# dfdazac/mpqe

Hardware: AMD Instinct MI355X
Metric: query-graphs/sec (encoder fwd+bwd) (higher is better)
Workload: dtype f32; 1 GPU; AIFB-shaped full query mix: 11 batches x B=512 per step (1/2/3-chain, 2x each of 2-inter, 3-inter, 3-inter_chain, 3-chain_inter), embed_dim=128, readout=mp, adaptive=True, num_layers=3 unshared, KG aifb (2601 entities, 89 typed relations); parallelism=single GPU

## Files before the change

### mpqe_amd/csrc/step.hip

```cpp
#include <stdio.h>
#include <stdlib.h>
#include <string.h>

#include <algorithm>
#include <memory>
#include <mutex>
#include <unordered_map>
#include <vector>

#include "grad_w_dma.h"
#include "rgcn_template_body.h"

#define STEP_MAX_LEVELS MPQE_STEP_MAX_LAYERS
#define CHAIN_MAX_GRAPHS (1 << 20)
#define UPLOAD_BYTES 2048

struct BatchDev {
    TmplArgs tp;
    int A, V, L, B;
    long long var_id[3];
    int anchor_tab[3];
    int target_tab;
    long long row_off, g_off, anchor_off;
    float weight;
// ... 956 lines not shown
__global__ __launch_bounds__(256) void adam_rows_kernel(const TouchHeader *__restrict__ th, const tkey_t *__restrict__ keys,
                                                        int D, RowAdamPtrs rp, float omb1, float omb2, float eps,
                                                        float neg_step_size, const int32_t *__restrict__ guard,
                                                        long long *__restrict__ applied) {
    if (guard && *guard != 0) return;
    if (applied && blockIdx.x == 0 && threadIdx.x == 0) *applied += 1;
    const int lpr = D / 4, per = 256 / lpr;
    const long long k = (long long)blockIdx.x * per + threadIdx.x / lpr;
    const int c = (threadIdx.x % lpr) * 4;
    if (k >= th->M) return;
    const tkey_t key = keys[k];
    if (key == TOUCH_INVALID || (k > 0 && keys[k - 1] == key)) return;
    const int tab = (int)(key >> th->row_bits);
    const long long off = (long long)(key & ((1ull << th->row_bits) - 1ull)) * D + c;
    float *p = rp.p[0], *m = rp.m[0], *v = rp.v[0];
    const float *g = rp.g[0];
#pragma unroll
    for (int t = 1; t < MPQE_STEP_MAX_MODES; ++t)
        if (t == tab) {
            p = rp.p[t];
            m = rp.m[t];
            v = rp.v[t];
            g = rp.g[t];
        }
    if (!p || !g || !m || !v) return;
    const f32x4 gg = gload4(g + off);
    f32x4 pp = *reinterpret_cast<f32x4 *>(p + off), mm = *reinterpret_cast<f32x4 *>(m + off);
    f32x4 vv = *reinterpret_cast<f32x4 *>(v + off);
#pragma unroll
    for (int e = 0; e < 4; ++e) {
        const float m_upd = __fmul_rn(__fsub_rn(gg[e], mm[e]), omb1);
        const float v_upd = __fmul_rn(__fsub_rn(__fmul_rn(gg[e], gg[e]), vv[e]), omb2);
        const float numer = __fadd_rn(m_upd, mm[e]);
        const float v_new = __fadd_rn(v_upd, vv[e]);
        const float denom = __fadd_rn(sqrtf(v_new), eps);
        mm[e] = __fadd_rn(mm[e], m_upd);
        vv[e] = v_new;
        pp[e] = __fadd_rn(pp[e], __fmul_rn(neg_step_size, __fdiv_rn(numer, denom)));
    }
    *reinterpret_cast<f32x4 *>(p + off) = pp;
    *reinterpret_cast<f32x4 *>(m + off) = mm;
    *reinterpret_cast<f32x4 *>(v + off) = vv;
}

extern "C" int64_t mpqe_step_touch_entries(const mpqe_step_batch_t *B, int nb) {
    if (!B || nb < 1 || nb > MPQE_STEP_MAX_BATCHES) return -1;
    return touch_entries(B, nb);
}

extern "C" size_t mpqe_rows_plan_bytes(int64_t n) { return n > 0 ? touch_layout(n, 0).total : 0; }
extern "C" size_t mpqe_rows_plan_workspace_bytes(int64_t n, int key_bits) {
    return n > 0 && key_bits > 0 && key_bits <= 64 ? touch_layout(n, key_bits).w_total : 0;
}
__global__ __launch_bounds__(256) void iota_kernel(int *__restrict__ v, long long n) {
    const long long i = (long long)blockIdx.x * 256 + threadIdx.x;
    if (i < n) v[i] = (int)i;
}
extern "C" int mpqe_rows_plan_build(const uint64_t *keys, int64_t n, int row_bits, int key_bits, void *plan,
                                    size_t plan_bytes, void *workspace, size_t workspace_bytes, void *stream) {
    if (!keys || !plan || !workspace || n <= 0 || n >= (1ll << 31) || row_bits <= 0 || key_bits <= row_bits || key_bits > 64)
        return MPQE_ERR_INVALID_ARG;
    const TouchLayout L = touch_layout(n, key_bits);
    if (plan_bytes < L.total || workspace_bytes < L.w_total) return MPQE_ERR_WORKSPACE;
    if ((uintptr_t)plan % 256 != 0 || (uintptr_t)workspace % 256 != 0) return MPQE_ERR_INVALID_ARG;
    hipStream_t s = as_stream(stream);
    char *tb = reinterpret_cast<char *>(plan), *wb = reinterpret_cast<char *>(workspace);
    TouchHeader th;
    memset(&th, 0, sizeof(th));
    th.M = n;
    th.row_bits = row_bits;
    th.key_bits = key_bits;
    upload(s, tb, &th, sizeof(th));
    int *vals = reinterpret_cast<int *>(wb + L.w_vals);
    hipLaunchKernelGGL(iota_kernel, dim3((unsigned)((n + 255) / 256)), dim3(256), 0, s, vals, (long long)n);
    if (radix_sort_pairs_own<tkey_t>(wb + L.w_tmp, reinterpret_cast<const tkey_t *>(keys), reinterpret_cast<tkey_t *>(tb + L.keys),
                                     (const int *)vals, reinterpret_cast<int *>(tb + L.perm), (long long)n, key_bits, s))
        return MPQE_ERR_LAUNCH;
    return mpqe_launch_status();
}
__global__ __launch_bounds__(256) void rows_sum_kernel(const char *__restrict__ plan, size_t o_keys, size_t o_perm,
                                                       const float *__restrict__ rows, int D, TablePtrs tabs, int store) {
    const TouchHeader *th = reinterpret_cast<const TouchHeader *>(plan);
    table_sum_block(th->M, th->row_bits, reinterpret_cast<const tkey_t *>(plan + o_keys),
                    reinterpret_cast<const int *>(plan + o_perm), rows, D, tabs, store, (long long)blockIdx.x);
}
extern "C" int mpqe_table_rows_sum(const void *plan, int64_t n, const float *rows, int64_t dim, float *const *table_grads,
                                   int num_modes, int store, void *stream) {
    if (!plan || !rows || !table_grads || n <= 0 || num_modes <= 0 || num_modes > MPQE_STEP_MAX_MODES)
        return MPQE_ERR_INVALID_ARG;
    if (dim <= 0 || dim % 4 != 0 || dim > 1024 || 256 % (dim / 4) != 0 || (uintptr_t)rows % 16 != 0) return MPQE_ERR_UNSUPPORTED;
    TablePtrs tabs;
    memset(&tabs, 0, sizeof(tabs));
    for (int m = 0; m < num_modes; ++m) {
        tabs.grad[m] = table_grads[m];
        if ((uintptr_t)table_grads[m] % 16 != 0) return MPQE_ERR_INVALID_ARG;
    }
    const TouchLayout L = touch_layout(n, 0);
    const long long per = 256 / (dim / 4);
    hipLaunchKernelGGL(rows_sum_kernel, dim3((unsigned)((n + per - 1) / per)), dim3(256), 0, as_stream(stream),
                       reinterpret_cast<const char *>(plan), L.keys, L.perm, rows, (int)dim, tabs, store);
    return mpqe_launch_status();
}

__global__ __launch_bounds__(256) void step_table_rows_kernel(const char *__restrict__ touch, size_t o_keys, size_t o_perm,
                                                              long long M, int row_bits, const float *__restrict__ DG, int D,
                                                              TablePtrs tabs, int store) {
    table_sum_block(M, row_bits, reinterpret_cast<const tkey_t *>(touch + o_keys), reinterpret_cast<const int *>(touch + o_perm),
                    DG, D, tabs, store, (long long)blockIdx.x, &reinterpret_cast<const TouchHeader *>(touch)->pad[0]);
}
extern "C" int mpqe_step_table_rows(const mpqe_step_params_t *P, const mpqe_step_batch_t *B, int nb, const mpqe_step_grads_t *G,
                                    const void *desc, void *workspace, size_t workspace_bytes, const void *touch, void *stream) {
    if (!P || !B || !G || !desc || !workspace || !touch || nb < 1 || nb > MPQE_STEP_MAX_BATCHES) return MPQE_ERR_INVALID_ARG;
    if ((uintptr_t)touch % 256 != 0 || (uintptr_t)workspace % 256 != 0) return MPQE_ERR_INVALID_ARG;
    std::shared_ptr<const CachedPlan> cached;
    if (plan_lookup(P, B, nb, nullptr, const_cast<void *>(desc), nullptr, &cached)) return MPQE_ERR_INVALID_ARG;
    const HostPlan &hp = cached->hp;
    if (!hp.chain || hp.touch_M <= 0) return MPQE_ERR_UNSUPPORTED;
    if (workspace_bytes < hp.total) return MPQE_ERR_WORKSPACE;
    const int D = P->dim;
    if (D % 4 != 0 || 256 % (D / 4) != 0) return MPQE_ERR_UNSUPPORTED;
    long long trows = 1;
    TablePtrs tabs;
    memset(&tabs, 0, sizeof(tabs));
    for (int m = 0; m < P->num_modes; ++m) {
        trows = std::max(trows, (long long)P->table_rows[m]);
        tabs.grad[m] = G->tables[m];
        tabs.rows[m] = P->table_rows[m];
        if (G->tables[m] && (uintptr_t)G->tables[m] % 16 != 0) return MPQE_ERR_INVALID_ARG;
    }
    const TouchLayout TL = touch_layout(hp.touch_M, 0);
    const long long per = 256 / (D / 4);
    const int store = ((P->flags & MPQE_STEP_SPARSE_TABLES) || (P->flags & MPQE_STEP_ZERO_GRADS)) ? 1 : 0;
    hipLaunchKernelGGL(step_table_rows_kernel, dim3((unsigned)((hp.touch_M + per - 1) / per)), dim3(256), 0, as_stream(stream),
                       reinterpret_cast<const char *>(touch), TL.keys, TL.perm, (long long)hp.touch_M, touch_bits(trows),
                       reinterpret_cast<const float *>(reinterpret_cast<const char *>(workspace) + hp.o_DG), D, tabs, store);
    return mpqe_launch_status();
}

static int adam_rows_launch(const void *touch, int64_t num_entries, float *const *params, const float *const *grads,
                            float *const *exp_avg, float *const *exp_avg_sq, int num_modes, int64_t dim, double lr,
                            double beta1, double beta2, double eps, int64_t step, const int32_t *guard, int64_t *applied,
                            void *stream) {
    if (!touch || num_entries <= 0 || !params || !grads || !exp_avg || !exp_avg_sq || step < 1) return MPQE_ERR_INVALID_ARG;
    if (num_modes <= 0 || num_modes > MPQE_STEP_MAX_MODES || dim <= 0 || dim % 4 != 0 || dim > 1024 || 256 % (dim / 4) != 0)
        return MPQE_ERR_UNSUPPORTED;
    if (!(beta1 >= 0. && beta1 < 1. && beta2 >= 0. && beta2 < 1.)) return MPQE_ERR_INVALID_ARG;
    const long long M = num_entries;
    RowAdamPtrs rp;
    memset(&rp, 0, sizeof(rp));
    for (int m = 0; m < num_modes; ++m) {
        rp.p[m] = params[m];
        rp.g[m] = grads[m];
        rp.m[m] = exp_avg[m];
        rp.v[m] = exp_avg_sq[m];
        if (((uintptr_t)rp.p[m] | (uintptr_t)rp.g[m] | (uintptr_t)rp.m[m] | (uintptr_t)rp.v[m]) % 16 != 0)
            return MPQE_ERR_INVALID_ARG;
    }
    const double bc1 = 1.0 - pow(beta1, (double)step), bc2 = 1.0 - pow(beta2, (double)step);
    const float neg_step = (float)(-(lr * sqrt(bc2) / bc1));
    const TouchLayout L = touch_layout(M, 0);
    const char *tb = reinterpret_cast<const char *>(touch);
    const long long per = 256 / (dim / 4);
    hipLaunchKernelGGL(adam_rows_kernel, dim3((unsigned)((M + per - 1) / per)), dim3(256), 0, as_stream(stream),
                       reinterpret_cast<const TouchHeader *>(tb), reinterpret_cast<const tkey_t *>(tb + L.keys), (int)dim, rp,
                       (float)(1.0 - beta1), (float)(1.0 - beta2), (float)eps, neg_step, guard,
                       reinterpret_cast<long long *>(applied));
    return mpqe_launch_status();
}

extern "C" int mpqe_adam_rows_step(const void *touch, int64_t num_entries, float *const *params,
                                   const float *const *grads, float *const *exp_avg, float *const *exp_avg_sq,
                                   int num_modes, int64_t dim, double lr, double beta1, double beta2, double eps,
                                   int64_t step, void *stream) {
    return adam_rows_launch(touch, num_entries, params, grads, exp_avg, exp_avg_sq, num_modes, dim, lr, beta1, beta2, eps,
                            step, nullptr, nullptr, stream);
}

extern "C" int mpqe_adam_rows_step_guarded(const void *touch, int64_t num_entries, float *const *params,
                                           const float *const *grads, float *const *exp_avg, float *const *exp_avg_sq,
                                           int num_modes, int64_t dim, double lr, double beta1, double beta2, double eps,
                                           int64_t step, const int32_t *guard, int64_t *applied, void *stream) {
    if (!guard) return MPQE_ERR_INVALID_ARG;
    return adam_rows_launch(touch, num_entries, params, grads, exp_avg, exp_avg_sq, num_modes, dim, lr, beta1, beta2, eps,
                            step, guard, applied, stream);
}

extern "C" int mpqe_l2_norms(const float *const *params, const int64_t *sizes, int count, const float *grad_out, float *out,
                             float *const *grads, void *stream) {
    if (!params || !sizes || count < 1 || count > 4 || (!out && !grads)) return MPQE_ERR_INVALID_ARG;
    RoRegArgs rr;
    memset(&rr, 0, sizeof(rr));
    for (int i = 0; i < count; ++i) {
        if (!params[i] || sizes[i] <= 0) return MPQE_ERR_INVALID_ARG;
        rr.p[i] = params[i];
        rr.n[i] = sizes[i];
        rr.g[i] = grads ? grads[i] : nullptr;
    }
    rr.coef = 1.f;
    rr.loss = out;
    rr.gscale = grad_out;
    hipLaunchKernelGGL(step_ro_reg_kernel, dim3(1), dim3(1024), 0, as_stream(stream), rr);
    return mpqe_launch_status();
}

static int D_ok_for_readout(int D) { return D % 4 == 0; }
static int readout_kin(const mpqe_step_params_t *P) {
    return P->readout == MPQE_READOUT_TARGETMLP ? 2 * P->dim : (P->readout == MPQE_READOUT_CONCAT ? P->num_layers * P->dim : P->dim);
}
// ... 42 lines not shown
```

### mpqe_amd/csrc/step_chain.h

```cpp
#pragma once
#include <type_traits>
#include "gemm_core.h"

#define CH_GB 16
#define CH_FIRST 1
#define CH_LAST 2
#define CH_LEVEL_END 4
#define CH_RELU 8
#define CH_MASK 16
#define CH_NOSTORE 32
#define CH_ADDG 64
#define CH_NOBIAS 128
#define CH_TSLOT_ON (1 << 20)
#define CH_MASK_LEVELS 4
#define CH_MAX_OPS 80
#define CH_MAX_CV 12

typedef float f32x2 __attribute__((ext_vector_type(2)));
typedef const f32x2 __attribute__((address_space(1))) * gvec2_ptr;
__device__ __forceinline__ f32x2 gload2(const float *p) { return *(gvec2_ptr)(p); }

struct ChainOp {
    unsigned char src, node, layer, level;
    int mat, flags;
// ... 964 lines not shown
#pragma unroll
            for (int cc = 0; cc < CC; ++cc) {
                q[cc] = h[A * CH_GB * LDX + sl + 16 * cc];
                arg[cc] = 0;
            }
        } else
#pragma unroll
        for (int cc = 0; cc < CC; ++cc) {
            const int col = sl + 16 * cc;
            float hn[4];
#pragma unroll
            for (int n = 0; n < 4; ++n) hn[n] = h[(n < N ? n : 0) * CH_GB * LDX + col];
            float sum = hn[0], best = hn[0];
            int am = 0;
#pragma unroll
            for (int n = 1; n < 4; ++n) {
                sum += n < N ? hn[n] : 0.f;
                const bool gt = n < N && hn[n] > best;
                best = gt ? hn[n] : best;
                am = gt ? n : am;
            }
            float tm = hn[0];
#pragma unroll
            for (int n = 1; n < 4; ++n) tm = n == A ? hn[n] : tm;
            q[cc] = readout == MPQE_READOUT_TM ? tm : (readout == MPQE_READOUT_SUM ? sum : best);
            arg[cc] = am;
        }
        if (ca.q_out && on) {
            float *qo = ca.q_out + (gi0 + i) * D;
#pragma unroll
            for (int cc = 0; cc < CC; ++cc) qo[sl + 16 * cc] = q[cc];
        }
        float ssp = 0.f, ssn = 0.f;
#pragma unroll
        for (int cc = 0; cc < CC; ++cc) {
            ssp += tp[cc] * tp[cc];
            ssn += tn[cc] * tn[cc];
        }
        ssp = gsum(ssp);
        ssn = gsum(ssn);
        const float ip0 = chain_rsq(ssp), in0 = chain_rsq(ssn);
        float dp = 0.f, dn = 0.f, qq = 0.f, pp = 0.f, nn = 0.f;
#pragma unroll
        for (int cc = 0; cc < CC; ++cc) {
            tp[cc] = pp_ ? tp[cc] * ip0 : 0.f;
            tn[cc] = pn_ ? tn[cc] * in0 : 0.f;
            dp += q[cc] * tp[cc];
            dn += q[cc] * tn[cc];
            qq += q[cc] * q[cc];
            pp += tp[cc] * tp[cc];
            nn += tn[cc] * tn[cc];
        }
        dp = gsum(dp);
        dn = gsum(dn);
        qq = gsum(qq);
        pp = gsum(pp);
        nn = gsum(nn);
        const float eps = ca.eps;
        const float rq = sqrtf(qq), rp = sqrtf(pp), rn = sqrtf(nn);
        const float nq = fmaxf(rq, eps), np_ = fmaxf(rp, eps), nn_ = fmaxf(rn, eps);
        const float sp = dp / (nq * np_), sn = dn / (nq * nn_);
        const float hv = ca.margin - (sp - sn);
        const long long gi = gi0 + i;
        const float term = on && hv > 0.f ? hv : 0.f;
        if (on && sl == 0) {
            ca.s_pos[gi] = sp;
            ca.s_neg[gi] = sn;
            ca.terms[gi] = term;
        }
        {
            float t4 = term + __shfl_xor(term, 16, 64);
            t4 += __shfl_xor(t4, 32, 64);
            if (lane == 0) S.red()[wave] = t4;
        }
        if (ca.backward) {
            const float act = hv >= 0.f ? b.weight / (float)b.B : 0.f;
            const float gsp = -act, gsn = act;
            const float inv_p = chain_rcp(nq * np_), inv_n = chain_rcp(nq * nn_);
            const float kq_ = rq > eps ? (gsp * sp + gsn * sn) * chain_rcp(nq * nq) : 0.f;
            const float ktp = rp > eps ? sp * chain_rcp(np_ * np_) : 0.f;
            const float ktn = rn > eps ? sn * chain_rcp(nn_ * nn_) : 0.f;
            const unsigned tmask = readout == MPQE_READOUT_SUM ? 0xFu : 1u << A;
            const unsigned liveL = b.live[RO ? L + 2 : L];
            float yg_p = 0.f, yg_n = 0.f;
#pragma unroll
            for (int cc = 0; cc < CC; ++cc) {
                const int col = sl + 16 * cc;
                const float gyp = gsp * (q[cc] * inv_p - ktp * tp[cc]);
                const float gyn = gsn * (q[cc] * inv_n - ktn * tn[cc]);
                yg_p += tp[cc] * gyp;
                yg_n += tn[cc] * gyn;
                float gq = gsp * tp[cc] * inv_p + gsn * tn[cc] * inv_n - kq_ * q[cc];
                if (RO) gq *= rscale;
                const unsigned takes = readout == MPQE_READOUT_MAX ? 1u << arg[cc] : tmask;
#pragma unroll
                for (int n = 0; n < 4; ++n) {
                    const float gv = (takes >> n) & 1u ? gq : 0.f;
                    if (n < N && ((liveL >> n) & 1u)) {
                        Xc[(n * CH_GB + i) * LDX + col] = gv;
                        if (on) GL[((long long)i * N + n) * D + col] = gv;
                    }
                }
            }
            yg_p = gsum(yg_p);
            yg_n = gsum(yg_n);
            float *gt = tabs.grad[b.target_tab];
            if (ca.DG && on) {
                float *dp_ = ca.DG + (ca.Manchor + ref.gi0 + i) * D, *dn_ = dp_ + ca.Gtot * D;
#pragma unroll
                for (int cc = 0; cc < CC; ++cc) {
                    const int col = sl + 16 * cc;
                    const float gyp = gsp * (q[cc] * inv_p - ktp * tp[cc]);
                    const float gyn = gsn * (q[cc] * inv_n - ktn * tn[cc]);
                    dp_[col] = pp_ ? (gyp - tp[cc] * yg_p) * ip0 : 0.f;
                    dn_[col] = pn_ ? (gyn - tn[cc] * yg_n) * in0 : 0.f;
                }
            } else if (gt && on) {
                const float *tb = tabs.table[b.target_tab];
#pragma unroll
                for (int cc = 0; cc < CC; ++cc) {
                    const int col = sl + 16 * cc;
                    const float gyp = gsp * (q[cc] * inv_p - ktp * tp[cc]);
                    const float gyn = gsn * (q[cc] * inv_n - ktn * tn[cc]);
                    if (CHAIN_DBG == 8) continue;
                    if (pp_) atomicAdd(gt + (pp_ - tb) + col, (gyp - tp[cc] * yg_p) * ip0);
                    if (pn_) atomicAdd(gt + (pn_ - tb) + col, (gyn - tn[cc] * yg_n) * in0);
                }
            }
        }
    }
    __syncthreads();
    if (tid == 0) {
        const float term = (S.red()[0] + S.red()[1]) + (S.red()[2] + S.red()[3]);
        if (ca.backward) ca.block_terms[ref.tb] = term;
        else agent_store(ca.block_terms + ref.tb, term);
    }
    if (!ca.backward) {
        chain_stamp(ca, 6);
        return;
    }
    chain_stamp(ca, 4);
    const int blk = g0 / CH_GB;
    for (int n = 0; n < N; ++n) {
        const int pr = b.lpart[n];
        if (pr < 0) continue;
        chain_colsum<NCB, KS, NW>(S, S.xs + cur * BUF, 1u << n, ng, ca.parts + (long long)(pr + blk) * D);
    }

    chain_run<NCB, KS, true, NW, RO>(S, nfwd, ref.bwd_count * IPO, N, ng, ca.GH + row0 * D, ca.level_stride, cur,
                                     ca.parts, blk);

    chain_stamp(ca, 5);
    if (ca.done) {
#ifndef MPQE_EMU
        asm volatile("s_waitcnt vmcnt(0)" ::: "memory");
#endif
        __syncthreads();
        if (tid == 0) {
            const unsigned inc = (unsigned)ca.done_inc[ref.done];
            const unsigned before = atomicAdd(ca.arrive + ref.done, 1u);
            if ((before + 1u) % inc == 0u) {
#ifndef MPQE_EMU
                __builtin_amdgcn_fence(__ATOMIC_RELEASE, "agent");
                asm volatile("s_waitcnt vmcnt(0)" ::: "memory");
#endif
                atomicAdd(ca.done + ref.done, inc);
            }
        }
    }
    if (four) {
        const float *Xc = S.xs + cur * BUF;
        const float *H0 = ca.H + row0 * D;
        const int nk = N * DB;
        const unsigned live0 = b.live[0];
        f32x4 y[4 * DB];
#pragma unroll
        for (int k = 0; k < 4 * DB; ++k) {
            const int f = tid + 256 * (k < nk ? k : 0);
            const int r = f / (D / 4), c4 = f - r * (D / 4);
            y[k] = gload4(H0 + (long long)(r < nrows ? r : 0) * D + 4 * c4);
        }
#pragma unroll
        for (int k = 0; k < 4 * DB; ++k) {
            const int f = tid + 256 * (k < nk ? k : 0);
            const int r = f / (D / 4), c4 = f - r * (D / 4);
            const int i = r / N, n = r - i * N;
            const bool on = k < nk && r < nrows && n < A && ((live0 >> n) & 1u);
            const f32x4 g = *reinterpret_cast<const f32x4 *>(Xc + (n * CH_GB + i) * LDX + 4 * c4);
            float yg = y[k][0] * g[0] + y[k][1] * g[1] + y[k][2] * g[2] + y[k][3] * g[3];
#pragma unroll
            for (int off = LPR >> 1; off >= 16; off >>= 1) yg += __shfl_xor(yg, off, 64);
            yg = chain_sum16(yg);
            if (ca.DG) {
                if (k < nk && r < nrows && n < A) {
                    const bool ok = on && S.rowp[r] != nullptr;
                    const float inv = ok ? S.nrm[r] : 0.f;
                    f32x4 o;
#pragma unroll
                    for (int e = 0; e < 4; ++e) o[e] = ok ? (g[e] - y[k][e] * yg) * inv : 0.f;
                    *reinterpret_cast<f32x4 *>(ca.DG + ((long long)ref.e0 + (long long)n * ref.B + i) * D + 4 * c4) = o;
                }
                continue;
            }
            float *gd = on ? S.gradp[r] : nullptr;
            if (gd && CHAIN_DBG != 7 && CHAIN_DBG != 8) {
                const float inv = S.nrm[r];
#pragma unroll
                for (int e = 0; e < 4; ++e) atomicAdd(gd + 4 * c4 + e, (g[e] - y[k][e] * yg) * inv);
            }
        }
    }
    chain_stamp(ca, 6);
#ifndef MPQE_EMU
    asm volatile("" ::"v"(wq[0]), "v"(wq[1]), "v"(wq[2]), "v"(wq[3]));
#else
    (void)wq;
#endif
}
```

### mpqe_amd/csrc/step_tail.h

```cpp
#pragma once

template <int MODE, int LDS_TILES = 4>
__device__ __forceinline__ void grad_w_block(const StepDev *__restrict__ sd, const WSource *__restrict__ src,
                                             int nsrc, const WBlock *__restrict__ block_start,
                                             const float *__restrict__ H, const float *__restrict__ GH,
                                             long long level_stride, float *__restrict__ slabs, int bid,
                                             int wblocks_total, float *smem, const GradPtrs &gp, bool zeroed,
                                             long long *dbg, int D, const PostArgs *po = nullptr, int tile_n = GT_BN,
                                             int nxcd = 8) {
    const int tiles_j = (D + tile_n - 1) / tile_n, tiles = tiles_j * ((D + GT_BM - 1) / GT_BM);
    const int nx = po ? po->na : nxcd;
    const int span = nx * tiles;
    int vb = bid;
    if (bid < (wblocks_total / span) * span) {
        const int grp = bid / span, r = bid - grp * span;
        vb = grp * span + (r % nx) * tiles + (r / nx);
    }
    const WBlock wk = block_start[vb];
    if (po) {
        if (threadIdx.x < 64) {
            const unsigned ep = *po->epoch_m + 1u;
            for (int c = wk.d0 + (int)threadIdx.x; c < wk.d0 + wk.dn; c += 64)
                uop_wait_until(po->done + c, ep * (unsigned)po->done_inc[c], po->err);
        }
// ... 59 lines not shown
        const int k = s.level_or_k;
        const long long g0 = (long long)blk * CH_GB;
        if (c < D)
            for (long long gi = g0 + rg; gi < g0 + CH_GB && gi < b.B; gi += 4)
                acc += g[(gi * b.tp.N + b.A + k) * D + c];
    }
    part[rg][cl] = acc;
    __syncthreads();
    if (rg == 0 && c < D)
        partial[(long long)(s.part_start + blk) * D + c] = (part[0][cl] + part[1][cl]) + (part[2][cl] + part[3][cl]);
}

__device__ __forceinline__ void anchor_bwd_block(const StepDev *__restrict__ sd, const TablePtrs &tabs,
                                                 const long long *__restrict__ node_map, long long map_len,
                                                 const long long *__restrict__ anchor_ids,
                                                 const float *__restrict__ G0,
                                                 const int *__restrict__ anchor_row_off, int nb, int bid) {
    const long long w = (long long)bid * 4 + (threadIdx.x >> 6);
    const int lane = threadIdx.x & 63;
    if (w >= anchor_row_off[nb]) return;
    const int bi = find_le(anchor_row_off, nb + 1, (int)w);
    const BatchDev &b = sd->b[bi];
    const long long lr = w - anchor_row_off[bi];
    const int n = (int)(lr / b.B);
    const long long g = lr - (long long)n * b.B;
    const int D = sd->D, tab = b.anchor_tab[n];
    float *gt = tabs.grad[tab];
    if (!gt || !((b.live[0] >> n) & 1u)) return;
    const long long row = table_row(node_map, map_len, anchor_ids[b.anchor_off + lr], tabs.rows[tab], nullptr);
    if (row < 0) return;
    const float *v = tabs.table[tab] + row * D;
    const float *gi = G0 + (b.row_off + g * b.tp.N + n) * D;
    float ss = 0.f, vg = 0.f;
    for (int c = lane; c < D; c += 64) {
        ss += v[c] * v[c];
        vg += v[c] * gi[c];
    }
    ss = wave_sum(ss);
    vg = wave_sum(vg);
    const float nrm = sqrtf(ss), inv = 1.f / nrm, ydotg = vg * inv;
    for (int c = lane; c < D; c += 64) atomicAdd(gt + row * D + c, (gi[c] - (v[c] / nrm) * ydotg) * inv);
}

#ifndef VEC_SLICES
#define VEC_SLICES 4
#endif
struct ReduceArgs {
    const RGroup *groups;
    int ngroups, D;
    GradPtrs gp;
    const float *slabs, *partial;
    int vec, zeroed;
    const StepDev *sd;
    const float *terms;
    float *loss;
    LossMeta lm;
    const float *bterms;
    const Rank1 *rank1;
    const float *VT;
    unsigned *epoch_b;
    const char *touch;
    size_t touch_keys, touch_perm;
    const float *DG;
    TablePtrs tabs;
    int table_store;
    long long touch_M;
    int touch_row_bits;
    int32_t *err;
    int nmat;
    const int *runs;
    unsigned *notify;
    unsigned notify_value;
};
__device__ __forceinline__ void reduce_block(const ReduceArgs &ra, int bx, int by, int gx, f32x4 (*part)[64]) {
    const RGroup *__restrict__ groups = ra.groups;
    const int ngroups = ra.ngroups, D = ra.D, vec = ra.vec, zeroed = ra.zeroed, table_store = ra.table_store;
    const GradPtrs &gp = ra.gp;
    const float *__restrict__ slabs = ra.slabs, *__restrict__ partial = ra.partial, *__restrict__ VT = ra.VT;
    const Rank1 *__restrict__ rank1 = ra.rank1;
    unsigned *epoch_b = ra.epoch_b;
    const char *__restrict__ touch = ra.touch;
    if (by > ngroups) {
        table_sum_block(ra.touch_M, ra.touch_row_bits, reinterpret_cast<const tkey_t *>(touch + ra.touch_keys),
                        reinterpret_cast<const int *>(touch + ra.touch_perm), ra.DG, D, ra.tabs, table_store & 1,
                        (long long)(by - ngroups - 1) * gx + bx, &reinterpret_cast<const TouchHeader *>(touch)->pad[0],
                        ra.runs, ra.runs ? ra.runs + ra.touch_M : nullptr);
        return;
    }
    if (by == ngroups) {
        if (bx == 0) {
            if (epoch_b && threadIdx.x == 0) {
                *epoch_b = *epoch_b + 1u;
                *(epoch_b - 16) = *(epoch_b - 16) + 1u;
                if (table_store & 2) *(epoch_b + 32) = *(epoch_b + 32) + 1u;
                *(epoch_b + 24) = 0u;
            }
            if (touch && threadIdx.x == 0 && reinterpret_cast<const TouchHeader *>(touch)->pad[0]) flag_error(ra.err, MPQE_FLAG_TOUCH_RETRY);
            if (ra.notify && threadIdx.x == 0) {
                ra.notify[1] = ra.err ? (unsigned)*ra.err : 0u;
#ifndef MPQE_EMU
                __builtin_amdgcn_fence(__ATOMIC_RELEASE, "");
#endif
                ra.notify[0] = ra.notify_value;
            }
            if (ra.lm.chain) loss_block_chain(ra.lm, ra.bterms, ra.loss, reinterpret_cast<float *>(part), 4);
            else loss_block(ra.sd, ra.terms, ra.loss, reinterpret_cast<float *>(part), 4);
        }
        return;
    }
    const RGroup g = groups[by];
    const bool wide = g.kind >= 4;
    const long long elems = (g.kind <= 1 || wide) ? (long long)D * D : D;
    if (g.kind >= 2 && !wide && vec && (256 % (D / 4)) == 0) {
        const int NS = (D % (4 * VEC_SLICES) == 0 && 256 % (D / 4 / VEC_SLICES) == 0 && (ra.nmat >= 0 || gx >= VEC_SLICES)) ? VEC_SLICES : 1;
        if (bx >= NS) return;
        const int LQ = D / 4 / NS, RG = 256 / LQ;
        const int c4 = bx * LQ + threadIdx.x % LQ, rg = threadIdx.x / LQ;
        const float *pv = partial + (long long)g.start * D + 4 * c4;
        f32x4 acc4 = {0.f, 0.f, 0.f, 0.f};
        for (int i = rg; i < g.count; i += RG * 8) {
            f32x4 v[8];
#pragma unroll
            for (int q = 0; q < 8; ++q) {
                const int k = i + RG * q;
                v[q] = gload4(pv + (long long)(k < g.count ? k : i) * D);
            }
#pragma unroll
            for (int q = 0; q < 8; ++q)
                if (i + RG * q < g.count) acc4 += v[q];
        }
        f32x4 *flat = &part[0][0];
        flat[threadIdx.x] = acc4;
        __syncthreads();
        const int cl = threadIdx.x % LQ;
        f32x4 t = acc4;
        if (rg < 4)
            for (int q = rg + 4; q < RG; q += 4) t += flat[q * LQ + cl];
        __syncthreads();
        if (rg < 4) flat[threadIdx.x] = t;
        __syncthreads();
        if (rg != 0) return;
        float *dstv = g.kind == 2 ? gp.bias[g.layer] : (gp.mode_emb ? gp.mode_emb + g.row * D : nullptr);
        if (!dstv) return;
        for (int q = 1; q < 4 && q < RG; ++q) t += flat[q * LQ + cl];
#pragma unroll
        for (int k = 0; k < 4; ++k) dstv[4 * c4 + k] = zeroed ? t[k] : dstv[4 * c4 + k] + t[k];
        return;
    }
    const int el = threadIdx.x & 63, sg = threadIdx.x >> 6;
    const long long idx = ((long long)bx * 64 + el) * 4;
    if ((long long)bx * 256 >= elems) return;
    f32x4 s = {0.f, 0.f, 0.f, 0.f};
    const float *p = ((g.kind <= 1 || wide) ? slabs : partial) + (long long)g.start * elems + idx;
    float *dst;
    if (g.kind == 0) dst = gp.basis[g.layer] ? gp.basis[g.layer] + g.row * elems : nullptr;
    else if (g.kind == 1) dst = gp.root[g.layer];
    else if (wide) {
        const long long cb = g.row & 255, nbk = g.row >> 8;
        dst = gp.root[g.layer] ? gp.root[g.layer] + (idx / D) * (nbk - 1) * D + cb * D : nullptr;
    }
    else if (g.kind == 2) dst = gp.bias[g.layer];
    else dst = gp.mode_emb ? gp.mode_emb + g.row * D : nullptr;
    const bool r1 = g.kind <= 1 && g.r1_count > 0 && vec && idx + 3 < elems && !(STEP_DBG & 2);
    const int ri = (int)(idx / D), rj = (int)(idx % D);
    Rank1 rk0[R1_CHUNK];
    float u0[R1_CHUNK];
    if (r1) {
// ... 233 lines not shown
```

### mpqe_amd/csrc/step_touch.h

```cpp
#pragma once
#include "radix_sort.h"

typedef unsigned long long tkey_t;
#define TOUCH_INVALID (~0ull)

#define TSORT_THREADS 256
#define TSORT_ROUNDS 8
#define TSORT_PER_BLOCK (TSORT_THREADS * TSORT_ROUNDS)
#define TSORT_MAX_BLOCKS 256
#define TSORT_MAX_ENTRIES ((long long)TSORT_MAX_BLOCKS * TSORT_PER_BLOCK)
static inline int tsort_rounds(long long M) { return M <= (long long)TSORT_MAX_BLOCKS * TSORT_THREADS * 4 ? 4 : TSORT_ROUNDS; }
static inline int tsort_blocks(long long M) {
    const long long per = (long long)TSORT_THREADS * tsort_rounds(M);
    return (int)((M + per - 1) / per);
}

struct TouchHeader {
    long long M;
    int row_bits, key_bits;
    int pad[12];
};
struct TouchLayout {
    size_t keys, perm, erow, total;
    size_t w_keys, w_vals, w_svals, w_hist, w_tmp, w_tmp_bytes, w_total;
// ... 257 lines not shown
        }
        if (p + 1 < passes) {
#pragma unroll
            for (int r = 0; r < TSORT_ROUNDS; ++r)
                if (r < R) {
                    tsort_st(dk + at[r], k[r]);
                    tsort_st(dv + at[r], v[r]);
                }
            bar += (unsigned)nblk;
            good = tsort_grid_barrier(sa.counter, bar, ok) && good;
            stamp();
#pragma unroll
            for (int r = 0; r < TSORT_ROUNDS; ++r)
                if (r < R) {
                    const int i = b * per_block + r * TSORT_THREADS + t;
                    k[r] = tsort_ld(dk + i);
                    v[r] = tsort_ld(dv + i);
                }
            dk = dk == sa.ka ? sa.kb : sa.ka;
            dv = dv == sa.va ? sa.vb : sa.va;
        } else {
#pragma unroll
            for (int r = 0; r < TSORT_ROUNDS; ++r)
                if (r < R && v[r] < (unsigned)M) {
                    sa.keys_out[at[r]] = k[r] == 0xffffffffu ? TOUCH_INVALID : (tkey_t)k[r];
                    sa.perm[at[r]] = (int)v[r];
                }
        }
    }
    if (sa.stamps && t == 0) sa.stamps[(long long)b * 8 + 7] = (long long)wall_clock64();
    if (t == 0 && (b == 0 || !good)) {
        TouchHeader th;
        memset(&th, 0, sizeof(th));
        th.M = M;
        th.row_bits = sa.row_bits;
        th.key_bits = sa.key_bits;
        if (b == 0 && good) *sa.th_out = th;
        else if (!good) {
            if (b == 0) *sa.th_out = th;
            __hip_atomic_store(&sa.th_out->pad[0], 1, __ATOMIC_RELAXED, __HIP_MEMORY_SCOPE_AGENT);
        }
    }
}
#else
__device__ __forceinline__ void tsort_block(const TSortArgs &sa, int b, unsigned *) {
    if (b != 0 || threadIdx.x != 0) return;
    const int M = sa.M;
    if (sa.fail) {
        TouchHeader th;
        memset(&th, 0, sizeof(th));
        th.M = M;
        th.row_bits = sa.row_bits;
        th.key_bits = sa.key_bits;
        th.pad[0] = 1;
        *sa.th_out = th;
        return;
    }
    std::vector<std::pair<tkey_t, int>> e((size_t)M);
    for (int i = 0; i < M; ++i) {
        int er;
        e[i].first = touch_key_of(*sa.tm, i, sa.anchor_ids, sa.targets, sa.negs, sa.node_map, sa.map_len, &er);
        e[i].second = i;
        if (sa.erow) sa.erow[i] = er;
    }
    std::stable_sort(e.begin(), e.end(), [](const std::pair<tkey_t, int> &x, const std::pair<tkey_t, int> &y) { return x.first < y.first; });
    for (int i = 0; i < M; ++i) {
        sa.keys_out[i] = e[i].first;
        sa.perm[i] = e[i].second;
    }
    TouchHeader th;
    memset(&th, 0, sizeof(th));
    th.M = M;
    th.row_bits = sa.row_bits;
    th.key_bits = sa.key_bits;
    *sa.th_out = th;
}
#endif
__global__ __launch_bounds__(TSORT_THREADS) void touch_sort_kernel(TSortArgs sa) {
    __shared__ unsigned smem[TSORT_LDS_WORDS];
    tsort_block(sa, (int)blockIdx.x, smem);
}

#define TS_AHEAD 8
template <class TabsT>
__device__ __forceinline__ void table_sum_block(long long M, int row_bits, const tkey_t *__restrict__ keys,
                                                const int *__restrict__ perm, const float *__restrict__ DG, int D,
                                                const TabsT &tabs, int store, long long block,
                                                const int *__restrict__ failed = nullptr,
                                                const int *__restrict__ runs = nullptr, const int *__restrict__ nruns = nullptr) {
    const int lpr = D / 4, per = 256 / lpr;
    long long k = block * per + threadIdx.x / lpr;
    const int c = (threadIdx.x % lpr) * 4;
    if (runs) {
        if (k >= (long long)*nruns) return;
        k = runs[k];
    }
    if (k >= M) return;
    const int bad = failed ? *failed : 0;
    const tkey_t key = keys[k];
    const tkey_t prev = k > 0 ? keys[k - 1] : TOUCH_INVALID;
    const long long p0 = perm ? (long long)perm[k] : k;
    tkey_t kk[TS_AHEAD];
    long long pj[TS_AHEAD];
#pragma unroll
    for (int q = 0; q < TS_AHEAD; ++q) {
        const long long j = k + 1 + q < M ? k + 1 + q : M - 1;
        kk[q] = keys[j];
        pj[q] = perm ? (long long)perm[j] : j;
    }
    if (bad || key == TOUCH_INVALID || (k > 0 && prev == key)) return;
    f32x4 acc = gload4(DG + p0 * D + c);
    {
        f32x4 v[TS_AHEAD];
        bool on[TS_AHEAD];
        bool more = true;
#pragma unroll
        for (int q = 0; q < TS_AHEAD; ++q) {
            more = more && k + 1 + q < M && kk[q] == key;
            on[q] = more;
            v[q] = more ? gload4(DG + pj[q] * D + c) : f32x4{0.f, 0.f, 0.f, 0.f};
        }
#pragma unroll
        for (int q = 0; q < TS_AHEAD; ++q)
            if (on[q]) acc += v[q];
        if (more) {
            for (long long j0 = k + 1 + TS_AHEAD; j0 < M; j0 += TS_AHEAD) {
                tkey_t k2[TS_AHEAD];
                long long p2[TS_AHEAD];
#pragma unroll
                for (int q = 0; q < TS_AHEAD; ++q) {
                    const long long j = j0 + q < M ? j0 + q : M - 1;
                    k2[q] = keys[j];
                    p2[q] = perm ? (long long)perm[j] : j;
                }
                f32x4 w[TS_AHEAD];
#pragma unroll
                for (int q = 0; q < TS_AHEAD; ++q) w[q] = gload4(DG + p2[q] * D + c);
                bool go = true;
#pragma unroll
                for (int q = 0; q < TS_AHEAD; ++q) {
                    go = go && j0 + q < M && k2[q] == key;
                    if (go) acc += w[q];
                }
                if (!go) break;
            }
        }
    }
    const int tab = (int)(key >> row_bits);
    const long long row = (long long)(key & ((1ull << row_bits) - 1ull));
    float *g = tabs.grad[0];
#pragma unroll
    for (int m = 1; m < MPQE_STEP_MAX_MODES; ++m)
        if (m == tab) g = tabs.grad[m];
    if (!g) return;
    f32x4 *dst = reinterpret_cast<f32x4 *>(g + row * D + c);
    if (store) *dst = acc;
    else *dst = *dst + acc;
}

#define TRUNS_EACH 8
#define TRUNS_PER (256 * TRUNS_EACH)
__device__ __forceinline__ void touch_runs_block(long long M, const tkey_t *__restrict__ keys, int *__restrict__ runs,
                                                 int *__restrict__ count, const int *__restrict__ failed, int *lds, int block) {
    const int tid = threadIdx.x;
    const int bad = failed ? *failed : 0;
    const long long base = (long long)block * TRUNS_PER;
    tkey_t key[TRUNS_EACH], prev[TRUNS_EACH];
#pragma unroll
    for (int q = 0; q < TRUNS_EACH; ++q) {
        const long long k = base + 256 * q + tid;
        key[q] = k < M ? keys[k] : TOUCH_INVALID;
        prev[q] = (k > 0 && k < M) ? keys[k - 1] : TOUCH_INVALID;
    }
    if (tid == 0) lds[0] = 0;
    __syncthreads();
    int c = 0;
#pragma unroll
    for (int q = 0; q < TRUNS_EACH; ++q) {
        const long long k = base + 256 * q + tid;
        c += (!bad && key[q] != TOUCH_INVALID && (k == 0 || prev[q] != key[q])) ? 1 : 0;
    }
    const int mine = c > 0 ? (int)atomicAdd(reinterpret_cast<unsigned *>(&lds[0]), (unsigned)c) : 0;
    __syncthreads();
    if (tid == 0) lds[1] = lds[0] > 0 ? (int)atomicAdd(reinterpret_cast<unsigned *>(count), (unsigned)lds[0]) : 0;
    __syncthreads();
    int at = lds[1] + mine;
#pragma unroll
    for (int q = 0; q < TRUNS_EACH; ++q) {
        const long long k = base + 256 * q + tid;
        if (!bad && key[q] != TOUCH_INVALID && (k == 0 || prev[q] != key[q])) runs[at++] = (int)k;
    }
}
```

Before: 87.35 million query-graphs/s.

## Defer L2-normalization backward projection from per-occurrence to per-unique-row table sum

The backward of the embedding row normalization (subtract the x·g component and scale by 1/||x||) was applied per occurrence when writing DG. It now runs once per unique touched table row inside table_sum_block, after the duplicate occurrences are summed, using the table row to recompute the norm. This works because the projection is linear in the gradient. The chain kernel now writes raw gradients and drops the reductions it used for the projection. The cost is an extra table-row read, an rsqrt and shuffle reductions in the sum kernel, plus a new D<=256 limit.

Result: no change. 87.22 million query-graphs/s (-0.1%).

```diff
diff --git a/mpqe_amd/csrc/step.hip b/mpqe_amd/csrc/step.hip
--- a/mpqe_amd/csrc/step.hip
+++ b/mpqe_amd/csrc/step.hip
@@ -1062,7 +1062,7 @@
                                                        const float *__restrict__ rows, int D, TablePtrs tabs, int store) {
     const TouchHeader *th = reinterpret_cast<const TouchHeader *>(plan);
     table_sum_block(th->M, th->row_bits, reinterpret_cast<const tkey_t *>(plan + o_keys),
-                    reinterpret_cast<const int *>(plan + o_perm), rows, D, tabs, store, (long long)blockIdx.x);
+                    reinterpret_cast<const int *>(plan + o_perm), rows, D, tabs, store, 0, (long long)blockIdx.x);
 }
 extern "C" int mpqe_table_rows_sum(const void *plan, int64_t n, const float *rows, int64_t dim, float *const *table_grads,
                                    int num_modes, int store, void *stream) {
@@ -1086,7 +1086,7 @@
                                                               long long M, int row_bits, const float *__restrict__ DG, int D,
                                                               TablePtrs tabs, int store) {
     table_sum_block(M, row_bits, reinterpret_cast<const tkey_t *>(touch + o_keys), reinterpret_cast<const int *>(touch + o_perm),
-                    DG, D, tabs, store, (long long)blockIdx.x, &reinterpret_cast<const TouchHeader *>(touch)->pad[0]);
+                    DG, D, tabs, store, 1, (long long)blockIdx.x, &reinterpret_cast<const TouchHeader *>(touch)->pad[0]);
 }
 extern "C" int mpqe_step_table_rows(const mpqe_step_params_t *P, const mpqe_step_batch_t *B, int nb, const mpqe_step_grads_t *G,
                                     const void *desc, void *workspace, size_t workspace_bytes, const void *touch, void *stream) {
@@ -1098,12 +1098,13 @@
     if (!hp.chain || hp.touch_M <= 0) return MPQE_ERR_UNSUPPORTED;
     if (workspace_bytes < hp.total) return MPQE_ERR_WORKSPACE;
     const int D = P->dim;
-    if (D % 4 != 0 || 256 % (D / 4) != 0) return MPQE_ERR_UNSUPPORTED;
+    if (D % 4 != 0 || D > 256 || 256 % (D / 4) != 0) return MPQE_ERR_UNSUPPORTED;
     long long trows = 1;
     TablePtrs tabs;
     memset(&tabs, 0, sizeof(tabs));
     for (int m = 0; m < P->num_modes; ++m) {
         trows = std::max(trows, (long long)P->table_rows[m]);
+        tabs.table[m] = P->tables[m];
         tabs.grad[m] = G->tables[m];
         tabs.rows[m] = P->table_rows[m];
         if (G->tables[m] && (uintptr_t)G->tables[m] % 16 != 0) return MPQE_ERR_INVALID_ARG;
diff --git a/mpqe_amd/csrc/step_chain.h b/mpqe_amd/csrc/step_chain.h
--- a/mpqe_amd/csrc/step_chain.h
+++ b/mpqe_amd/csrc/step_chain.h
@@ -1070,14 +1070,9 @@
             const float ktn = rn > eps ? sn * chain_rcp(nn_ * nn_) : 0.f;
             const unsigned tmask = readout == MPQE_READOUT_SUM ? 0xFu : 1u << A;
             const unsigned liveL = b.live[RO ? L + 2 : L];
-            float yg_p = 0.f, yg_n = 0.f;
 #pragma unroll
             for (int cc = 0; cc < CC; ++cc) {
                 const int col = sl + 16 * cc;
-                const float gyp = gsp * (q[cc] * inv_p - ktp * tp[cc]);
-                const float gyn = gsn * (q[cc] * inv_n - ktn * tn[cc]);
-                yg_p += tp[cc] * gyp;
-                yg_n += tn[cc] * gyn;
                 float gq = gsp * tp[cc] * inv_p + gsn * tn[cc] * inv_n - kq_ * q[cc];
                 if (RO) gq *= rscale;
                 const unsigned takes = readout == MPQE_READOUT_MAX ? 1u << arg[cc] : tmask;
@@ -1090,9 +1085,17 @@
                     }
                 }
             }
-            yg_p = gsum(yg_p);
-            yg_n = gsum(yg_n);
             float *gt = tabs.grad[b.target_tab];
+            float yg_p = 0.f, yg_n = 0.f;
+            if (!ca.DG) {
+#pragma unroll
+                for (int cc = 0; cc < CC; ++cc) {
+                    yg_p += tp[cc] * (gsp * (q[cc] * inv_p - ktp * tp[cc]));
+                    yg_n += tn[cc] * (gsn * (q[cc] * inv_n - ktn * tn[cc]));
+                }
+                yg_p = gsum(yg_p);
+                yg_n = gsum(yg_n);
+            }
             if (ca.DG && on) {
                 float *dp_ = ca.DG + (ca.Manchor + ref.gi0 + i) * D, *dn_ = dp_ + ca.Gtot * D;
 #pragma unroll
@@ -1100,8 +1103,8 @@
                     const int col = sl + 16 * cc;
                     const float gyp = gsp * (q[cc] * inv_p - ktp * tp[cc]);
                     const float gyn = gsn * (q[cc] * inv_n - ktn * tn[cc]);
-                    dp_[col] = pp_ ? (gyp - tp[cc] * yg_p) * ip0 : 0.f;
-                    dn_[col] = pn_ ? (gyn - tn[cc] * yg_n) * in0 : 0.f;
+                    dp_[col] = pp_ ? gyp : 0.f;
+                    dn_[col] = pn_ ? gyn : 0.f;
                 }
             } else if (gt && on) {
                 const float *tb = tabs.table[b.target_tab];
@@ -1123,6 +1126,9 @@
         if (ca.backward) ca.block_terms[ref.tb] = term;
         else agent_store(ca.block_terms + ref.tb, term);
     }
+#ifdef MPQE_EMU
+    __syncthreads();
+#endif
     if (!ca.backward) {
         chain_stamp(ca, 6);
         return;
@@ -1156,7 +1162,23 @@
             }
         }
     }
-    if (four) {
+    if (four && ca.DG) {
+        const float *Xc = S.xs + cur * BUF;
+        const int nk = N * DB;
+        const unsigned live0 = b.live[0];
+#pragma unroll
+        for (int k = 0; k < 4 * DB; ++k) {
+            const int f = tid + 256 * (k < nk ? k : 0);
+            const int r = f / (D / 4), c4 = f - r * (D / 4);
+            const int i = r / N, n = r - i * N;
+            if (k < nk && r < nrows && n < A) {
+                const bool ok = ((live0 >> n) & 1u) && S.rowp[r] != nullptr;
+                const f32x4 g = *reinterpret_cast<const f32x4 *>(Xc + (n * CH_GB + i) * LDX + 4 * c4);
+                *reinterpret_cast<f32x4 *>(ca.DG + ((long long)ref.e0 + (long long)n * ref.B + i) * D + 4 * c4) =
+                    ok ? g : f32x4{0.f, 0.f, 0.f, 0.f};
+            }
+        }
+    } else if (four) {
         const float *Xc = S.xs + cur * BUF;
         const float *H0 = ca.H + row0 * D;
         const int nk = N * DB;
@@ -1179,17 +1201,6 @@
 #pragma unroll
             for (int off = LPR >> 1; off >= 16; off >>= 1) yg += __shfl_xor(yg, off, 64);
             yg = chain_sum16(yg);
-            if (ca.DG) {
-                if (k < nk && r < nrows && n < A) {
-                    const bool ok = on && S.rowp[r] != nullptr;
-                    const float inv = ok ? S.nrm[r] : 0.f;
-                    f32x4 o;
-#pragma unroll
-                    for (int e = 0; e < 4; ++e) o[e] = ok ? (g[e] - y[k][e] * yg) * inv : 0.f;
-                    *reinterpret_cast<f32x4 *>(ca.DG + ((long long)ref.e0 + (long long)n * ref.B + i) * D + 4 * c4) = o;
-                }
-                continue;
-            }
             float *gd = on ? S.gradp[r] : nullptr;
             if (gd && CHAIN_DBG != 7 && CHAIN_DBG != 8) {
                 const float inv = S.nrm[r];
diff --git a/mpqe_amd/csrc/step_tail.h b/mpqe_amd/csrc/step_tail.h
--- a/mpqe_amd/csrc/step_tail.h
+++ b/mpqe_amd/csrc/step_tail.h
@@ -165,7 +165,7 @@
     const char *__restrict__ touch = ra.touch;
     if (by > ngroups) {
         table_sum_block(ra.touch_M, ra.touch_row_bits, reinterpret_cast<const tkey_t *>(touch + ra.touch_keys),
-                        reinterpret_cast<const int *>(touch + ra.touch_perm), ra.DG, D, ra.tabs, table_store & 1,
+                        reinterpret_cast<const int *>(touch + ra.touch_perm), ra.DG, D, ra.tabs, table_store & 1, 1,
                         (long long)(by - ngroups - 1) * gx + bx, &reinterpret_cast<const TouchHeader *>(touch)->pad[0],
                         ra.runs, ra.runs ? ra.runs + ra.touch_M : nullptr);
         return;
diff --git a/mpqe_amd/csrc/step_touch.h b/mpqe_amd/csrc/step_touch.h
--- a/mpqe_amd/csrc/step_touch.h
+++ b/mpqe_amd/csrc/step_touch.h
@@ -363,10 +363,17 @@
 }
 
 #define TS_AHEAD 8
+__device__ __forceinline__ float touch_rsq(float x) {
+#ifdef MPQE_EMU
+    return 1.f / sqrtf(x);
+#else
+    return __builtin_amdgcn_rsqf(x);
+#endif
+}
 template <class TabsT>
 __device__ __forceinline__ void table_sum_block(long long M, int row_bits, const tkey_t *__restrict__ keys,
                                                 const int *__restrict__ perm, const float *__restrict__ DG, int D,
-                                                const TabsT &tabs, int store, long long block,
+                                                const TabsT &tabs, int store, int project, long long block,
                                                 const int *__restrict__ failed = nullptr,
                                                 const int *__restrict__ runs = nullptr, const int *__restrict__ nruns = nullptr) {
     const int lpr = D / 4, per = 256 / lpr;
@@ -390,6 +397,18 @@
         pj[q] = perm ? (long long)perm[j] : j;
     }
     if (bad || key == TOUCH_INVALID || (k > 0 && prev == key)) return;
+    const int tab = (int)(key >> row_bits);
+    const long long row = (long long)(key & ((1ull << row_bits) - 1ull));
+    float *g = tabs.grad[0];
+    const float *tv = tabs.table[0];
+#pragma unroll
+    for (int m = 1; m < MPQE_STEP_MAX_MODES; ++m)
+        if (m == tab) {
+            g = tabs.grad[m];
+            tv = tabs.table[m];
+        }
+    if (!g || (project && !tv)) return;
+    const f32x4 x = project ? gload4(tv + row * D + c) : f32x4{0.f, 0.f, 0.f, 0.f};
     f32x4 acc = gload4(DG + p0 * D + c);
     {
         f32x4 v[TS_AHEAD];
@@ -427,13 +446,27 @@
             }
         }
     }
-    const int tab = (int)(key >> row_bits);
-    const long long row = (long long)(key & ((1ull << row_bits) - 1ull));
-    float *g = tabs.grad[0];
-#pragma unroll
-    for (int m = 1; m < MPQE_STEP_MAX_MODES; ++m)
-        if (m == tab) g = tabs.grad[m];
-    if (!g) return;
+    if (project) {
+        float ss = x[0] * x[0] + x[1] * x[1] + x[2] * x[2] + x[3] * x[3];
+        float xg = x[0] * acc[0] + x[1] * acc[1] + x[2] * acc[2] + x[3] * acc[3];
+        int off = lpr >> 1;
+        for (; off >= 16; off >>= 1) {
+            ss += __shfl_xor(ss, off, 64);
+            xg += __shfl_xor(xg, off, 64);
+        }
+        if (off == 8) {
+            ss = chain_sum16(ss);
+            xg = chain_sum16(xg);
+        } else {
+            for (; off >= 1; off >>= 1) {
+                ss += __shfl_xor(ss, off, 64);
+                xg += __shfl_xor(xg, off, 64);
+            }
+        }
+        const float inv = touch_rsq(ss), s = inv * (inv * xg);
+#pragma unroll
+        for (int e = 0; e < 4; ++e) acc[e] = (acc[e] - x[e] * s) * inv;
+    }
     f32x4 *dst = reinterpret_cast<f32x4 *>(g + row * D + c);
     if (store) *dst = acc;
     else *dst = *dst + acc;
```
